# pingooio/pingoo

Measured on AMD Instinct MI355X. Metric: requests/sec matched (whole node), 1k-rule WAF, higher is better.
Workload: dtype u8

## Files before the change

include/pwaf.h:

```cpp
#ifndef PWAF_H
#define PWAF_H

#include <stddef.h>
#include <stdint.h>

#ifdef __cplusplus
extern "C" {
#endif

#define PWAF_ABI_VERSION 4u

#define PWAF_OK 0
#define PWAF_E_INVALID_ARG (-1)
#define PWAF_E_SYNTAX (-2)
#define PWAF_E_UNSUPPORTED (-3)
#define PWAF_E_LIST (-4)
#define PWAF_E_DEVICE (-5)
#define PWAF_E_BATCH (-6)
#define PWAF_E_NOMEM (-7)
#define PWAF_E_BUSY (-8)
#define PWAF_W_PARTIAL 1

#define PWAF_ACTION_ALLOW 0u
#define PWAF_ACTION_BLOCK 1u
// ... 275 lines not shown
    float ms;
    uint64_t alg_bytes;
} pwaf_kernel_time;
int pwaf_engine_set_profiling(pwaf_engine *, int on);
int pwaf_engine_kernel_times(pwaf_engine *, pwaf_kernel_time *out, int cap);

typedef struct pwaf_stats {
    uint32_t n_rules, n_atoms, n_scan_atoms, n_numeric_atoms;
    uint32_t n_dfa_groups, n_dfa_states_total, max_dfa_states, dfa_table_bytes_total;
    uint32_t n_ip_lists, ipset_trie_nodes, geo_trie_nodes, n_dnf_literals;
    uint32_t n_warnings, n_filtered_groups ,
        n_gated_groups ,
        n_confirm_literals ;
} pwaf_stats;
int pwaf_engine_stats(const pwaf_engine *, pwaf_stats *out);
int pwaf_engine_rule_errors(pwaf_engine *, uint64_t *counts, size_t n_rules);
int pwaf_engine_residual_mode(const pwaf_engine *);
const char *pwaf_engine_residual_fallback(const pwaf_engine *);
size_t pwaf_program_residual_source(const pwaf_program *, int kind, char *buf, size_t cap);
long pwaf_program_residual_compile(const pwaf_program *, const char *arch, char *err, size_t err_len);
int pwaf_program_confirm_field(const pwaf_program *, uint32_t group, const uint8_t *bytes, size_t len, uint32_t arena_offset,
                               uint16_t *atoms, size_t cap, size_t *n_atoms, int *flagged, int *walk);
int pwaf_engine_address_tables(const pwaf_engine *, uint32_t out[8]);
int pwaf_program_stats(const pwaf_program *, pwaf_stats *out);

size_t pwaf_derive_path(const uint8_t *uri_path, size_t len);
void pwaf_derive_user_agent(const uint8_t *hdr, size_t len, int present, size_t *out_start, size_t *out_len);
void pwaf_derive_host(const uint8_t *uri_host, size_t uri_host_len, int uri_host_present,
                      const uint8_t *host_hdr, size_t host_hdr_len, int host_hdr_present,
                      int *out_from_header, size_t *out_start, size_t *out_len);

const char *pwaf_last_error(void);
uint32_t pwaf_abi_version(void);

#ifdef __cplusplus
}
#endif
#endif
```

pingoo_amd/_abi.py:

```python
import ctypes as C

ABI_VERSION = 4

OK = 0
E_INVALID_ARG = -1
E_SYNTAX = -2
E_UNSUPPORTED = -3
E_LIST = -4
E_DEVICE = -5
E_BATCH = -6
E_NOMEM = -7
E_BUSY = -8

ACTION_ALLOW, ACTION_BLOCK, ACTION_CAPTCHA, ACTION_BYPASS = 0, 1, 2, 3
RULE_NONE = 0xFFFFFFFF
RULE_UA_GATE = 0xFFFFFFFE
RULE_CAPTCHA_ENDPOINT = 0xFFFFFFFD
RULE_ACTION_BLOCK, RULE_ACTION_CAPTCHA = 1, 2

LIST_STRING, LIST_INT, LIST_IP = 0, 1, 2
OPT_NO_UA_GATE, OPT_NO_CAPTCHA_BYPASS, OPT_NO_PREFILTER, OPT_STRICT, OPT_FILTER_STRIDE2, OPT_LENIENT, OPT_NO_RESIDUAL, OPT_GLOBAL_VERDICT_TABLES, OPT_NO_CONFIRM, OPT_NO_RESIDUAL_JIT = 1, 2, 4, 8, 16, 32, 64, 128, 512, 1024
OPT_DENSE_VERDICT, OPT_TINY_VERDICT_SLOTS, OPT_NO_DIR_SUMMARY, OPT_SPARSE_VERDICT, OPT_EAGER_CMP, OPT_NO_DENSE_SWITCH = 2048, 4096, 8192, 16384, 32768, 65536
OPT_GEO_ANSWERS = 256
OPT_RULE_HITS = 131072
W_PARTIAL = 1
MEM_HOST, MEM_DEVICE = 0, 1
FLAG_CAPTCHA_VERIFIED = 1
N_FIELDS = 5
FIELD_NAMES = ("host", "url", "path", "method", "user_agent")
ARENA_PAD = 16
ADDRESS_TABLE_FIELDS = ("escapes", "n_vals", "has_summary", "shift", "common", "packed", "classes", "sets")
GEO_ANSWER_TABLE_FIELDS = ("has_table", "escapes", "n_vals", "has_summary", "shift", "common", "records", "zero")


class RuleDesc(C.Structure):
    _fields_ = [
        ("name", C.c_char_p),
        ("expression", C.c_char_p),
        ("actions", C.POINTER(C.c_uint8)),
        ("n_actions", C.c_uint32),
        ("reserved", C.c_uint32),
    ]


class ListDesc(C.Structure):
    _fields_ = [
        ("name", C.c_char_p),
        ("type", C.c_uint32),
        ("n_items", C.c_uint32),
        ("items", C.POINTER(C.c_char_p)),
    ]


class GeoipEntry(C.Structure):
# ... 173 lines not shown
```

pingoo_amd/csrc/dirtable.h:

```cpp
#pragma once
#include <cstddef>
#include <cstdint>
#include <unordered_map>
#include <vector>

namespace pwaf {
namespace dirtable {

static constexpr uint32_t kChunkWords = 32;
static constexpr size_t kEntries = (size_t)1 << 24;

struct Compressed {
    std::vector<uint32_t> chunks;
    std::vector<uint32_t> vals;
    std::vector<uint32_t> summary;
    uint32_t shift = 0, common = 0;
};

inline void compress(const uint32_t *d24, bool no_summary, Compressed &out) {
    out.chunks.assign((size_t)65536 * kChunkWords, 0);
    out.vals.clear();
    out.summary.clear();
    out.shift = out.common = 0;
    for (uint32_t x = 0; x < 65536; x++) {
        const uint32_t *en = &d24[(size_t)x << 8];
        for (uint32_t w = 0; w < 8; w++) {
            uint32_t *rec = &out.chunks[(size_t)x * kChunkWords + 4 * w];
            uint32_t bm = 0, n_starts = 0;
            for (uint32_t j = 32 * w; j < 32 * w + 32; j++)
                if (j == 0 || en[j] != en[j - 1]) {
                    bm |= 1u << (j & 31);
                    if (n_starts == 1) rec[3] = (uint32_t)out.vals.size();
                    if (n_starts == 0) rec[2] = en[j];
                    else out.vals.push_back(en[j]);
                    n_starts++;
                }
            rec[0] = bm;
            rec[1] = w ? en[32 * w - 1] : 0u;
        }
    }
    if (out.vals.empty()) out.vals.push_back(0);
    if (no_summary) return;
    std::unordered_map<uint32_t, uint64_t> run_len;
    for (size_t x = 0; x < kEntries;) {
        size_t y = x + 1;
        while (y < kEntries && d24[y] == d24[x]) y++;
// ... 4 lines not shown
    uint64_t best_len = 0;
    for (const auto &kv : run_len)
        if (kv.second > best_len || (kv.second == best_len && kv.first < common)) { common = kv.first; best_len = kv.second; }
    double best_cost = 1e9;
    uint32_t best_shift = 0;
    std::vector<uint32_t> best_bits;
    for (uint32_t shift = 0; shift <= 4; shift++) {
        const size_t n_blk = kEntries >> shift;
        std::vector<uint32_t> bits(n_blk / 32, 0);
        uint64_t set = 0;
        for (size_t b = 0; b < n_blk; b++) {
            bool other = false;
            for (size_t j = b << shift; j < ((b + 1) << shift) && !other; j++) other = d24[j] != common;
            if (other) { bits[b >> 5] |= 1u << (b & 31); set++; }
        }
        const double cost = (double)set / (double)n_blk + (double)(n_blk / 8) / (8.0 * 1024 * 1024);
        if (cost < best_cost && set * 2 <= n_blk) { best_cost = cost; best_shift = shift; best_bits.swap(bits); }
    }
    if (!best_bits.empty()) {
        out.summary.swap(best_bits);
        out.shift = best_shift;
        out.common = common;
    }
}

}
}
```

pingoo_amd/csrc/engine.cpp:

```cpp
#include <hip/hip_runtime_api.h>

#include <cstdio>
#include <algorithm>
#include <cstring>
#include <map>
#include <memory>
#include <mutex>
#include <string>
#include <type_traits>
#include <unordered_map>
#include <vector>

#include "dirtable.h"
#include "georec.h"
#include "frontend.h"
#include "kernels.h"
#include "lscan_split.h"
#include "program.h"
#include "records.h"

using namespace pwaf;

struct pwaf_program {
    std::unique_ptr<Program> p;
// ... 230 lines not shown
    uint32_t cmp_vars = 0;
    uint32_t cc_words = 1, n_cmp_atoms = 0, n_bit_atoms = 0, n_trig = 0, n_lazy = 0;
    DevBuf lazy_atoms;
    std::vector<uint32_t> lazy_vars;
    uint32_t n_short = 0;
    int short_field = -1;
    DevBuf short_atoms;
    uint32_t class_words = 1, acmp_words = 0, geo_default = 0, n_classes = 1;
    DevBuf class_rows, dir_esc, leaf_root, geo_leaf_root;
    std::vector<uint32_t> host_cc_masks, host_iu_masks1;
    std::vector<std::pair<uint32_t, uint32_t>> host_acmp;
    std::vector<int64_t> host_iu_vals1;
    DevBuf iu_vals[2], iu_masks[2];
    uint32_t iu_n[2] = {0, 0}, iu_words[2] = {1, 1};
    DevBuf ip_root4, ip_root6, ip_nodes, geo_root4, geo_root6, geo_nodes, geo_recs;
    std::mutex mu;
    std::mutex prof_mu;
    DevBuf residual_errors;
    std::string residual_note;
    JitKernel residual_jit;
    DevBuf residual_blob, geo_rec_root4, geo_rec_root6, geo_rec_nodes;
    DevBuf pass_base, colmask, dir24 , dir_chunks, dir_vals, dir_summary;
    uint32_t dir_sum_shift = 0, dir_common = 0;
    uint32_t dir_n_esc = 0, dir_n_vals = 0;
    bool geo_answers = false;
    DevBuf georec_chunks, georec_vals, georec_summary;
    uint32_t georec_shift = 0, georec_common = 0, georec_n_esc = 0, georec_n_vals = 0;
    uint32_t n_need = 0;
    uint32_t n_visit = 0;
    std::vector<double> mean_len;
    uint32_t n_ungated = 0, n_gated = 0, n_filtered = 0;
    std::vector<uint8_t> owns_factors;
    uint32_t n_gap = 0;
    std::vector<uint32_t> lscan_launches[2];
    DevBuf pass_table;
    std::vector<uint32_t> hlen_fields;
    uint32_t n_fields = PWAF_N_FIELDS;
    int profiling = 0;
    std::vector<hipEvent_t> ev;
    std::vector<pwaf_kernel_time> times;
    std::vector<std::pair<size_t, size_t>> time_ev;
    size_t n_timed = 0;
    uint32_t n_cus = 256;
};

namespace {
// ... 247 lines not shown
}

void set_trie_args(const pwaf_engine *e, VerdictArgs &v) {
    const Program &P = *e->prog.p;
    const uint32_t *leaf = (const uint32_t *)e->leaf_root.p;
    v.ip_root4 = P.ipset_trie.root4.empty() ? leaf : (const uint32_t *)e->ip_root4.p;
    v.ip_root6 = P.ipset_trie.root6.empty() ? leaf : (const uint32_t *)e->ip_root6.p;
    v.ip_nodes = (const uint32_t *)e->ip_nodes.p;
    v.set_masks = (const uint32_t *)e->set_masks.p;
    v.set_words = P.set_words;
    v.n_ip_lists = P.n_ip_lists;
    const uint32_t *geo_leaf = (const uint32_t *)e->geo_leaf_root.p;
    v.geo_root4 = P.geo_trie.root4.empty() ? geo_leaf : (const uint32_t *)e->geo_root4.p;
    v.geo_root6 = P.geo_trie.root6.empty() ? geo_leaf : (const uint32_t *)e->geo_root6.p;
    v.geo_nodes = (const uint32_t *)e->geo_nodes.p;
    v.has_geo = P.has_geo ? 1u : 0u;
    v.dir24 = (const uint32_t *)e->dir24.p;
    v.dir_chunks = (const uint32_t *)e->dir_chunks.p;
    v.dir_vals = (const uint32_t *)e->dir_vals.p;
    v.dir_esc = (const uint2 *)e->dir_esc.p;
    v.dir_summary = (const uint32_t *)e->dir_summary.p;
    v.dir_sum_shift = e->dir_sum_shift;
    v.dir_common = e->dir_common;
    v.class_rows = (const uint32_t *)e->class_rows.p;
    v.class_words = e->class_words;
    v.acmp_words = e->acmp_words;
    v.geo_default = e->geo_default;
    const size_t n_sets = P.set_words ? P.set_masks.size() / P.set_words : 1;
    v.ipres_packed = (e->n_classes <= 65536u && n_sets <= 65536u) ? 1u : 0u;
}

void set_georec_args(const pwaf_engine *e, GeoRecArgs &g) {
    g.has_geo = e->prog.p->has_geo ? 1u : 0u;
    g.root4 = (const uint32_t *)e->geo_rec_root4.p;
    g.root6 = (const uint32_t *)e->geo_rec_root6.p;
    g.nodes = (const uint32_t *)e->geo_rec_nodes.p;
    g.recs = (const GeoRec *)e->geo_recs.p;
    g.chunks = (const uint32_t *)e->georec_chunks.p;
    g.vals = (const uint32_t *)e->georec_vals.p;
    g.summary = (const uint32_t *)e->georec_summary.p;
    g.sum_shift = e->georec_shift;
    g.common = e->georec_common;
    g.n_cus = e->n_cus;
}
int need_geo_answers(const pwaf_engine *e, const char *fn) {
    if (e->geo_answers) return PWAF_OK;
// ... 1491 lines not shown
        if (P.has_geo && P.residual_needs_geo) {
            const std::vector<uint32_t> leaf0(65536, TRIE_LEAF);
            UP(geo_rec_root4, (P.geo_trie.root4.empty() ? leaf0 : P.geo_trie.root4))
            UP(geo_rec_root6, (P.geo_trie.root6.empty() ? leaf0 : P.geo_trie.root6))
            UP(geo_rec_nodes, P.geo_trie.nodes)
            UP(geo_recs, P.geo_recs)
        }
    }
#undef UP
    if (P.flags & PWAF_OPT_GEO_ANSWERS) {
        e->geo_answers = true;
        const std::vector<uint32_t> leaf0(65536, TRIE_LEAF);
        if (!e->geo_rec_root4.p) {
            if ((rc = upload(e->geo_rec_root4, P.geo_trie.root4.empty() ? leaf0 : P.geo_trie.root4)) || (rc = upload(e->geo_rec_root6, P.geo_trie.root6.empty() ? leaf0 : P.geo_trie.root6)) ||
                (rc = upload(e->geo_rec_nodes, P.geo_trie.nodes)))
                return dev_fail(rc);
            const std::vector<GeoRec> def{GeoRec{0u, (uint16_t)('X' | ('X' << 8)), 0u}};
            if ((rc = upload(e->geo_recs, P.geo_recs.empty() ? def : P.geo_recs))) return dev_fail(rc);
        }
        if (P.has_geo && !P.geo_trie.root4.empty()) {
            std::vector<uint32_t> d24;
            e->georec_n_esc = georec::flatten(P.geo_trie.root4.data(), P.geo_trie.nodes.data(), d24);
            dirtable::Compressed ct;
            dirtable::compress(d24.data(), (P.flags & PWAF_OPT_NO_DIR_SUMMARY) != 0, ct);
            if ((rc = upload(e->georec_chunks, ct.chunks)) || (rc = upload(e->georec_vals, ct.vals))) return dev_fail(rc);
            if (!ct.summary.empty()) {
                if ((rc = upload(e->georec_summary, ct.summary))) return dev_fail(rc);
                e->georec_shift = ct.shift;
                e->georec_common = ct.common;
            }
            e->georec_n_vals = (uint32_t)ct.vals.size();
        }
    }
    if ((P.has_geo && !P.geo_trie.root4.empty()) || (P.n_ip_lists && !P.ipset_trie.root4.empty())) {
        VerdictArgs tv{};
        set_trie_args(e.get(), tv);
        DevBuf cnt;
        if ((rc = cnt.reserve(4))) return dev_fail(rc);
        uint32_t n_esc = 0;
        bool ok = hipMemset(cnt.p, 0, 4) == hipSuccess && launch_dir24(tv, nullptr, nullptr, cnt.p, nullptr) == 0 &&
                  hipMemcpy(&n_esc, cnt.p, 4, hipMemcpyDeviceToHost) == hipSuccess;
        if (ok) ok = e->dir24.reserve((size_t)4 << 24) == PWAF_OK && e->dir_esc.reserve((size_t)std::max(1u, n_esc) * 8) == PWAF_OK;
        if (ok) ok = hipMemset(cnt.p, 0, 4) == hipSuccess && launch_dir24(tv, e->dir24.p, e->dir_esc.p, cnt.p, nullptr) == 0 && hipDeviceSynchronize() == hipSuccess;
        cnt.release();
        if (!ok) { fail(PWAF_E_DEVICE, "DIR-24 table build failed"); return dev_fail(PWAF_E_DEVICE); }
        {
            std::vector<uint32_t> d24((size_t)1 << 24);
            if (hipMemcpy(d24.data(), e->dir24.p, d24.size() * 4, hipMemcpyDeviceToHost) != hipSuccess) { fail(PWAF_E_DEVICE, "DIR-24 download failed"); return dev_fail(PWAF_E_DEVICE); }
            static_assert(dirtable::kChunkWords == kDirChunkWords, "dirtable.h and kernels.h disagree on the record layout");
            dirtable::Compressed ct;
            dirtable::compress(d24.data(), (P.flags & PWAF_OPT_NO_DIR_SUMMARY) != 0, ct);
            if ((rc = upload(e->dir_chunks, ct.chunks)) || (rc = upload(e->dir_vals, ct.vals))) return dev_fail(rc);
            if (!ct.summary.empty()) {
                if ((rc = upload(e->dir_summary, ct.summary))) return dev_fail(rc);
                e->dir_sum_shift = ct.shift;
                e->dir_common = ct.common;
            }
            e->dir_n_esc = n_esc;
            e->dir_n_vals = (uint32_t)ct.vals.size();
            e->dir24.release();
        }
    }
    if (hipDeviceSynchronize() != hipSuccess) { fail(PWAF_E_DEVICE, "device synchronize failed after table upload"); return dev_fail(PWAF_E_DEVICE); }
    *out = e.release();
    return partial;
}

void pwaf_engine_destroy(pwaf_engine *e) {
    if (!e) return;
    for (auto &g : e->groups) { for (DevBuf *b : {&g.tab, &g.classmap, &g.special, &g.list_off, &g.list, &g.ftable, &g.c_head, &g.c_entries, &g.c_bytes, &g.c_classes}) b->release(); g.fl.release(); g.rt.release(); }
    for (DevBuf *b : {&e->num_atoms, &e->lazy_atoms, &e->bit_atoms, &e->trig_off, &e->trig_rules, &e->always_rules, &e->iu_vals[0], &e->iu_vals[1], &e->iu_masks[0], &e->iu_masks[1], &e->country_luts, &e->rules, &e->lits,
                      &e->set_masks, &e->ip_root4, &e->ip_root6, &e->ip_nodes, &e->geo_root4, &e->geo_root6, &e->geo_nodes, &e->geo_recs, &e->residual_blob, &e->residual_errors, &e->geo_rec_root4, &e->geo_rec_root6, &e->geo_rec_nodes, &e->pass_base, &e->colmask, &e->dir24, &e->dir_chunks, &e->dir_vals, &e->dir_summary, &e->class_rows,
                      &e->dir_esc, &e->leaf_root, &e->geo_leaf_root, &e->pass_table, &e->georec_chunks, &e->georec_vals, &e->georec_summary})
        b->release();
    if (e->residual_jit.module) {
        int cur = -1;
        const bool have = hipGetDevice(&cur) == hipSuccess;
        (void)hipSetDevice(e->device);
        jit_release(e->residual_jit);
        if (have) (void)hipSetDevice(cur);
    }
    for (auto &c : e->ctx) c->release();
    for (auto ev : e->ev) (void)hipEventDestroy(ev);
    delete e;
}

int pwaf_engine_residual_mode(const pwaf_engine *e) {
    if (!e || e->prog.p->n_residual == 0) return 0;
    return e->residual_jit.function ? 2 : 1;
}
const char *pwaf_engine_residual_fallback(const pwaf_engine *e) { return e ? e->residual_note.c_str() : ""; }
int pwaf_engine_address_tables(const pwaf_engine *e, uint32_t out[8]) {
    if (!e || !out) return fail(PWAF_E_INVALID_ARG, "pwaf_engine_address_tables: NULL argument");
    const Program &P = *e->prog.p;
    VerdictArgs v{};
    set_trie_args(e, v);
    out[0] = e->dir_n_esc;
    out[1] = e->dir_chunks.p ? e->dir_n_vals : 0u;
    out[2] = e->dir_summary.p ? 1u : 0u;
    out[3] = e->dir_sum_shift;
    out[4] = e->dir_common;
    out[5] = v.ipres_packed;
    out[6] = e->n_classes;
    out[7] = P.set_words ? (uint32_t)(P.set_masks.size() / P.set_words) : 1u;
    return PWAF_OK;
}
int pwaf_engine_geo_answer_tables(const pwaf_engine *e, uint32_t out[8]) {
    if (!e || !out) return fail(PWAF_E_INVALID_ARG, "pwaf_engine_geo_answer_tables: NULL argument");
    if (int rc = need_geo_answers(e, "pwaf_engine_geo_answer_tables")) return rc;
    out[0] = e->georec_chunks.p ? 1u : 0u;
    out[1] = e->georec_n_esc;
    out[2] = e->georec_chunks.p ? e->georec_n_vals : 0u;
    out[3] = e->georec_summary.p ? 1u : 0u;
    out[4] = e->georec_shift;
    out[5] = e->georec_common;
    out[6] = (uint32_t)std::max<size_t>(1, e->prog.p->geo_recs.size());
    out[7] = 0;
    return PWAF_OK;
}
size_t pwaf_program_residual_source(const pwaf_program *p, int kind, char *buf, size_t cap) {
    if (!p || p->p->n_residual == 0) return 0;
    std::string text, why;
    const std::vector<uint8_t> &blob = p->p->residual_blob;
    if (!(kind == 0 ? rvm_specialize(blob.data(), blob.size(), text, why) : rvm_jit_program(blob.data(), blob.size(), text, why))) {
        (void)fail(PWAF_E_UNSUPPORTED, why);
        return 0;
    }
// ... 914 lines not shown
```

pingoo_amd/csrc/kernels.h:

```cpp
#pragma once
#include <cstdint>
#include <string>
#include <vector>

#include "program.h"

namespace pwaf {

static constexpr int kMaxPasses = 250;
static constexpr int kVerdictPre = 12;
static constexpr uint32_t kGapLists = 32;
static constexpr uint32_t kMaxHeaderLens = 8;
static constexpr uint32_t kDirChunkWords = 32;

static constexpr uint32_t REC_OVERFLOW = 0x80000000u;
struct PoolEntry {
    uint32_t atom;
    uint32_t next;
};

struct SpecialCell {
    uint32_t next_off;
    uint32_t emit;
};
// ... 278 lines not shown
    uint32_t lazy_var[4], n_lazy_var;
    const uint32_t *bit_col;
    const int64_t *iu_vals[2];
    const uint32_t *iu_masks[2];
    uint32_t iu_n[2], iu_words[2];
    const uint32_t *country_masks;
    uint32_t cc_words;
    const DevRule *rules;
    uint32_t n_rules;
    const uint32_t *lits;
    uint32_t n_lits, n_trig;
    const uint32_t *trig_off;
    const uint16_t *trig_rules;
    const uint32_t *always_rules;
    const uint32_t *ip_root4, *ip_root6, *ip_nodes;
    const uint32_t *set_masks;
    uint32_t set_words;
    uint32_t n_ip_lists;
    const uint32_t *geo_root4, *geo_root6, *geo_nodes;
    const uint32_t *dir24;
    const uint32_t *dir_chunks, *dir_vals;
    const uint32_t *dir_summary;
    uint32_t dir_sum_shift, dir_common;
    const uint2 *dir_esc;
    const uint32_t *class_rows;
    uint32_t class_words;
    uint32_t acmp_words;
    uint32_t geo_default;
    uint32_t *ipres;
    uint32_t ipres_packed;
    uint32_t has_geo;
    uint4 *gpairs;
    uint32_t *ghdr;
    uint32_t pair_stride;
    uint32_t attr_blocks;
    pwaf_verdict *out;
    unsigned long long *counts;
    uint32_t *match_idx;
    uint32_t *n_matches;
    pwaf_rule_hit *hits;
    uint32_t hits_cap;
    uint32_t *n_hits;
    unsigned long long *rule_hits;
};

int launch_scan(const ScanArgs &a, void *stream);
struct GatedTable {
    const ListScanArgs *g;
    uint32_t count;
    uint32_t debug;
};
struct ListShape {
    uint32_t threads, hot_bytes, wg_per_cu;
};
ListShape list_shape(uint32_t variant);
uint32_t list_hot_bytes(const ListShape &shape);
int launch_scan_gated(const ListScanArgs *host, uint32_t count, const ListScanArgs *dev, uint32_t *plan, const ListShape &shape, void *stream);
int launch_verdict(const VerdictArgs &a, void *stream);
int launch_ipres(const VerdictArgs &a, void *stream);
int launch_attr(const VerdictArgs &a, void *stream);
int launch_dir24(const VerdictArgs &a, void *out , void *esc, void *esc_count, void *stream);
struct GeoRecArgs {
    const uint8_t *ip, *ip_is_v6;
    const uint32_t *asn;
    const uint16_t *country;
    uint32_t n, has_geo;
    const uint32_t *root4, *root6, *nodes;
    const GeoRec *recs;
    const uint32_t *chunks, *vals, *summary;
    uint32_t sum_shift, common;
    uint32_t n_cus;
    uint2 *out;
};
int launch_georec(const GeoRecArgs &a, void *stream);
uint32_t scan_lds_bytes(uint32_t n_hot, uint32_t stride, uint32_t n_gate_atoms);
struct VerdictShape {
    uint32_t waves, lds_bytes, lds_tables;
    uint32_t sparse, v_cap, per_cu;
};
VerdictShape verdict_shape(uint32_t n_cols, uint32_t n_rules, uint32_t n_trig, uint32_t n_lits, bool force_global = false, int mode = 3, uint32_t n_passes = 0);
uint32_t verdict_blocks_sp(const VerdictShape &sh, uint32_t n_cus);

// ... 2 lines not shown
```

pingoo_amd/csrc/kernels.hip:

```cpp
#include <hip/hip_runtime.h>

#include <cstdlib>
#include <mutex>
#include <set>

#include "confirm.h"
#include "utf8.h"
#include "kernels.h"
#include "residual.h"

namespace pwaf {

static constexpr int kScanThreads = 1024;
static constexpr int kScanWaves = kScanThreads / 64;
static constexpr uint32_t kNone = 0xFFFFFFFFu;

#define PWAF_LDS __attribute__((address_space(3)))
#define PWAF_GLOBAL __attribute__((address_space(1)))
typedef const PWAF_LDS uint16_t *lds_u16_ptr;
typedef const PWAF_GLOBAL uint16_t *glb_u16_ptr;
typedef const PWAF_LDS uint32_t *lds_u32_ptr;
typedef const PWAF_LDS uint8_t *lds_u8_ptr;
typedef unsigned int u32x4 __attribute__((ext_vector_type(4)));
typedef u32x4 u32x4_u __attribute__((aligned(1)));
// ... 2744 lines not shown
        __builtin_amdgcn_fence(__ATOMIC_ACQ_REL, "wavefront");
        if (HITS && q_n != 0 && ++q_k == 0x10000u) q_flush();
        cur = nxt;
    }
    if (HITS && a.n_hits != nullptr) q_flush();
    __syncthreads();
    unsigned long long *tally = reinterpret_cast<unsigned long long *>(lds);
    if (lane == 0) {
        tally[wave * 4 + PWAF_ACTION_ALLOW] = cnt_allow;
        tally[wave * 4 + PWAF_ACTION_BLOCK] = cnt_block;
        tally[wave * 4 + PWAF_ACTION_CAPTCHA] = cnt_captcha;
        tally[wave * 4 + PWAF_ACTION_BYPASS] = cnt_bypass;
    }
    __syncthreads();
    if (a.counts != nullptr && tid < 4) {
        unsigned long long sum = 0;
        for (uint32_t wv = 0; wv < n_waves; wv++) sum += tally[wv * 4 + tid];
        if (sum) atomicAdd(&a.counts[tid], sum);
    }
}

static constexpr uint32_t DIR_ESCAPE = 0x80000000u;

template <bool PACKED>
__global__ __launch_bounds__(256) void ipres_kernel(VerdictArgs a) {
    constexpr uint32_t U = 4;
    const bool from_row = a.asn == nullptr;
#ifdef PWAF_PROFILING
    const bool dir = a.dir_chunks != nullptr && !((a.debug_skip >> 16) & 1u);
    const bool skip_v6 = (a.debug_skip >> 17) & 1u, skip_v4 = (a.debug_skip >> 16) & 1u;
#else
    const bool dir = a.dir_chunks != nullptr;
    constexpr bool skip_v6 = false, skip_v4 = false;
#endif
    const uint32_t T = gridDim.x * 256u;
    for (uint32_t i0 = blockIdx.x * 256u + threadIdx.x; i0 < a.n; i0 += T * U) {
        uint32_t idx[U], ipw[U][4], eg[U], ei[U], k[U];
        bool live[U], v6[U], geo_walk[U], chunked[U];
        uint4 raw[U];
        uint32_t v6b[U];
#pragma unroll
        for (uint32_t u = 0; u < U; u++) {
            idx[u] = i0 + u * T;
            live[u] = idx[u] < a.n;
            const uint32_t j = live[u] ? idx[u] : i0;
            raw[u] = *reinterpret_cast<const uint4 *>(a.ip + (size_t)j * 16);
            v6b[u] = a.ip_is_v6[j];
        }
        uint32_t first[U], top16[U];
#pragma unroll
        for (uint32_t u = 0; u < U; u++) {
            ipw[u][0] = raw[u].x; ipw[u][1] = raw[u].y; ipw[u][2] = raw[u].z; ipw[u][3] = raw[u].w;
            v6[u] = v6b[u] != 0;
            geo_walk[u] = false;
            if (from_row && a.has_geo) {
                if (!v6[u]) {
                    const uint32_t b0 = ipw[u][0] & 0xFFu;
                    geo_walk[u] = !(b0 == 127u || (b0 & 0xF0u) == 0xE0u);
                } else {
                    const bool loopback = ipw[u][0] == 0 && ipw[u][1] == 0 && ipw[u][2] == 0 && ipw[u][3] == 0x01000000u;
                    geo_walk[u] = !(loopback || (ipw[u][0] & 0xFFu) == 0xFFu);
                }
            }
            top16[u] = (ip_byte(ipw[u], 0) << 8) | ip_byte(ipw[u], 1);
            eg[u] = ei[u] = TRIE_LEAF;
            chunked[u] = !v6[u] && dir;
            first[u] = 0;
            if (!chunked[u] && !(v6[u] ? skip_v6 : skip_v4)) {
                if (geo_walk[u]) eg[u] = (v6[u] ? a.geo_root6 : a.geo_root4)[top16[u]];
                if (a.n_ip_lists) ei[u] = (v6[u] ? a.ip_root6 : a.ip_root4)[top16[u]];
            }
        }
        uint32_t look[U];
#pragma unroll
        for (uint32_t u = 0; u < U; u++) {
            look[u] = chunked[u] ? 1u : 0u;
            if (chunked[u] && a.dir_summary != nullptr) {
                const uint32_t blk = ((top16[u] << 8) | ip_byte(ipw[u], 2)) >> a.dir_sum_shift;
                look[u] = (a.dir_summary[blk >> 5] >> (blk & 31u)) & 1u;
            }
        }
        uint4 rec4[U];
#pragma unroll
        for (uint32_t u = 0; u < U; u++) {
            rec4[u] = make_uint4(0u, 0u, 0u, 0u);
            if (look[u]) rec4[u] = *reinterpret_cast<const uint4 *>(a.dir_chunks + (size_t)top16[u] * kDirChunkWords + 4u * (ip_byte(ipw[u], 2) >> 5));
        }
        uint32_t e24[U];
#pragma unroll
        for (uint32_t u = 0; u < U; u++) {
            e24[u] = a.dir_common;
            if (look[u]) {
                const uint32_t rank = (uint32_t)__builtin_popcount(rec4[u].x & (0xFFFFFFFFu >> (31u - (ip_byte(ipw[u], 2) & 31u))));
                e24[u] = rank == 0 ? rec4[u].y : rank == 1 ? rec4[u].z : a.dir_vals[rec4[u].w + rank - 2u];
            }
        }
#pragma unroll
        for (uint32_t u = 0; u < U; u++) {
            k[u] = 2;
            if (!v6[u] && dir) {
// ... 394 lines not shown
    const uint32_t x = blockIdx.x * 256 + threadIdx.x;
    if (x >= (1u << 24)) return;
    uint32_t eg = a.geo_root4[x >> 8];
    if (!(eg & TRIE_LEAF)) eg = a.geo_nodes[(size_t)eg * 256 + (x & 0xFFu)];
    uint32_t ei = a.ip_root4[x >> 8];
    if (!(ei & TRIE_LEAF)) ei = a.ip_nodes[(size_t)ei * 256 + (x & 0xFFu)];
    const uint32_t vg = eg & ~TRIE_LEAF, vi = ei & ~TRIE_LEAF;
    if ((eg & ei & TRIE_LEAF) && vg < 65536u && vi < 32768u) {
        if (out) out[x] = vg | (vi << 16);
        return;
    }
    const uint32_t idx = atomicAdd(esc_count, 1u);
    if (esc) {
        esc[idx] = make_uint2(eg, ei);
        out[x] = DIR_ESCAPE | idx;
    }
}

int launch_dir24(const VerdictArgs &a, void *out, void *esc, void *esc_count, void *stream) {
    hipLaunchKernelGGL(dir24_kernel, dim3((1u << 24) / 256), dim3(256), 0, (hipStream_t)stream, a, (uint32_t *)out, (uint2 *)esc, (uint32_t *)esc_count);
    return (int)hipGetLastError();
}

int launch_ipres(const VerdictArgs &a, void *stream) {
    if (a.n == 0) return 0;
#ifdef PWAF_PROFILING
    static const uint32_t forced = getenv("PWAF_IPRES_BLOCKS") ? (uint32_t)atoi(getenv("PWAF_IPRES_BLOCKS")) : 0u;
#else
    const uint32_t forced = 0;
#endif
    const uint32_t blocks = std::min<uint32_t>((a.n + 255) / 256, forced ? forced : 8 * std::max(1u, a.attr_blocks));
    if (a.ipres_packed) hipLaunchKernelGGL(ipres_kernel<true>, dim3(blocks), dim3(256), 0, (hipStream_t)stream, a);
    else hipLaunchKernelGGL(ipres_kernel<false>, dim3(blocks), dim3(256), 0, (hipStream_t)stream, a);
    return (int)hipGetLastError();
}

int launch_georec(const GeoRecArgs &a, void *stream) {
    if (a.n == 0) return 0;
    const uint32_t blocks = std::min<uint32_t>((a.n + 255) / 256, 8 * std::max(1u, a.n_cus));
    hipLaunchKernelGGL(georec_kernel, dim3(blocks), dim3(256), 0, (hipStream_t)stream, a);
    return (int)hipGetLastError();
}

int launch_attr(const VerdictArgs &a, void *stream) {
    if (a.n == 0) return 0;
#ifdef PWAF_PROFILING
    static const uint32_t forced = getenv("PWAF_ATTR_BLOCKS") ? (uint32_t)atoi(getenv("PWAF_ATTR_BLOCKS")) : 0u;
#else
    const uint32_t forced = 0;
#endif
    const uint32_t blocks = std::min<uint32_t>((a.n_groups + 3) / 4, forced ? forced : 6 * std::max(1u, a.attr_blocks));
    const bool small = a.set_words <= 4 && a.cc_words <= 2 && a.iu_words[0] <= 1 && a.iu_words[1] <= 1 && a.acmp_words <= 1;
    if (a.ipres_packed && small) hipLaunchKernelGGL((attr_kernel<true, true>), dim3(blocks), dim3(256), 0, (hipStream_t)stream, a);
    else if (a.ipres_packed) hipLaunchKernelGGL((attr_kernel<true, false>), dim3(blocks), dim3(256), 0, (hipStream_t)stream, a);
    else if (small) hipLaunchKernelGGL((attr_kernel<false, true>), dim3(blocks), dim3(256), 0, (hipStream_t)stream, a);
    else hipLaunchKernelGGL((attr_kernel<false, false>), dim3(blocks), dim3(256), 0, (hipStream_t)stream, a);
// ... 142 lines not shown
```

pingoo_amd/engine.py:

```python
from __future__ import annotations

import ctypes as C
import enum
import ipaddress
import os
from dataclasses import dataclass, field
from typing import Dict, Iterable, List, Optional, Sequence, Tuple

import numpy as np

from . import _abi
from .batch import GEO_DTYPE, RULE_HIT_DTYPE, VERDICT_DTYPE, Request, RequestBatch

_LIB = None
_LIB_PATH = os.path.join(os.path.dirname(os.path.abspath(__file__)), f"libpwaf_{os.environ['PWAF_LIB_VARIANT']}.so" if os.environ.get("PWAF_LIB_VARIANT") else "libpwaf.so")


class PwafError(RuntimeError):
    def __init__(self, code: int, message: str, rule_index: Optional[int] = None):
        super().__init__(f"[{code}] {message}")
        self.code = code
        self.message = message
        self.rule_index = rule_index

# ... 95 lines not shown
    L.pwaf_batcher_destroy.argtypes = [vp]
    L.pwaf_batcher_destroy.restype = None
    L.pwaf_evaluate_records.argtypes = [vp, vp, C.c_size_t, vp, C.c_uint32, vp, vp]
    L.pwaf_async_create.argtypes = [vp, C.c_uint32, C.c_uint32, C.c_uint32, C.POINTER(vp)]
    L.pwaf_async_submit.argtypes = [vp, C.POINTER(_abi.Request), C.c_uint64]
    L.pwaf_async_poll.argtypes = [vp, C.POINTER(_abi.Completion), C.c_size_t]
    L.pwaf_async_poll.restype = C.c_size_t
    L.pwaf_async_fd.argtypes = [vp]
    L.pwaf_async_flush.argtypes = [vp]
    L.pwaf_async_stats.argtypes = [vp, C.POINTER(C.c_uint64), C.POINTER(C.c_uint64), C.POINTER(C.c_uint64)]
    L.pwaf_async_destroy.argtypes = [vp]
    L.pwaf_async_destroy.restype = None
    L.pwaf_geoip_lookup.argtypes = [vp, vp, vp, C.c_uint32, C.c_uint32, vp, vp]
    L.pwaf_evaluate_batch_geo.argtypes = [vp, C.POINTER(_abi.Batch), vp, vp, vp]
    L.pwaf_evaluate_device_geo.argtypes = [vp, C.POINTER(_abi.Batch), vp, vp, vp, vp, vp, vp]
    L.pwaf_evaluate_batch_hits.argtypes = [vp, C.POINTER(_abi.Batch), vp, vp, vp, C.c_uint32, vp, vp]
    L.pwaf_evaluate_device_hits.argtypes = [vp, C.POINTER(_abi.Batch), vp, vp, vp, vp, vp, C.c_uint32, vp, vp, vp]
    L.pwaf_evaluate_records_geo.argtypes = [vp, vp, C.c_size_t, vp, C.c_uint32, vp, vp, vp]
    L.pwaf_evaluate_one_geo.argtypes = [vp, C.POINTER(_abi.Request), C.POINTER(_abi.Verdict), C.POINTER(_abi.Geo)]
    L.pwaf_async_create_geo.argtypes = [vp, C.c_uint32, C.c_uint32, C.c_uint32, C.POINTER(vp)]
    L.pwaf_async_poll_geo.argtypes = [vp, C.POINTER(_abi.Completion), C.POINTER(_abi.Geo), C.c_size_t]
    L.pwaf_async_poll_geo.restype = C.c_size_t
    L.pwaf_engine_geo_answer_tables.argtypes = [vp, C.POINTER(C.c_uint32)]
    L.pwaf_geoip_from_mmdb.argtypes = [C.c_char_p, C.c_size_t, C.POINTER(C.POINTER(_abi.GeoipEntry)), C.POINTER(C.c_size_t)]
    L.pwaf_geoip_from_file_image.argtypes = [C.c_char_p, C.c_char_p, C.c_size_t, C.POINTER(C.POINTER(_abi.GeoipEntry)), C.POINTER(C.c_size_t)]
    L.pwaf_zstd_decompress.argtypes = [C.c_char_p, C.c_size_t, C.POINTER(C.c_void_p), C.POINTER(C.c_size_t)]
    L.pwaf_buffer_free.argtypes = [C.c_void_p]
    L.pwaf_buffer_free.restype = None
    L.pwaf_geoip_free.argtypes = [C.POINTER(_abi.GeoipEntry)]
    L.pwaf_geoip_free.restype = None
    L.pwaf_list_parse_csv.argtypes = [C.c_char_p, C.c_size_t, C.POINTER(C.POINTER(C.c_char_p)), C.POINTER(C.c_size_t)]
    L.pwaf_list_free.argtypes = [C.POINTER(C.c_char_p), C.c_size_t]
    L.pwaf_list_free.restype = None
    L.pwaf_engine_kernel_times.argtypes = [vp, C.POINTER(_abi.KernelTime), C.c_int]
    L.pwaf_derive_path.argtypes = [C.c_char_p, C.c_size_t]
    L.pwaf_derive_path.restype = C.c_size_t
    L.pwaf_derive_user_agent.argtypes = [C.c_char_p, C.c_size_t, C.c_int, C.POINTER(C.c_size_t), C.POINTER(C.c_size_t)]
    L.pwaf_derive_user_agent.restype = None
    L.pwaf_derive_host.argtypes = [C.c_char_p, C.c_size_t, C.c_int, C.c_char_p, C.c_size_t, C.c_int, C.POINTER(C.c_int), C.POINTER(C.c_size_t), C.POINTER(C.c_size_t)]
    L.pwaf_derive_host.restype = None
    if L.pwaf_abi_version() != _abi.ABI_VERSION:
        raise ImportError("libpwaf.so ABI version mismatch: rebuild with `python -m pingoo_amd.build --force`")
    _LIB = L
    return L


# ... 193 lines not shown
            self._h = None

    def __del__(self):
        self.close()

    @property
    def program(self) -> CompiledProgram:
        return CompiledProgram._borrow(lib().pwaf_engine_program(self._h))

    @property
    def residual_mode(self) -> int:
        return int(lib().pwaf_engine_residual_mode(self._h))

    @property
    def residual_fallback(self) -> str:
        return (lib().pwaf_engine_residual_fallback(self._h) or b"").decode(errors="replace")

    def address_tables(self) -> dict:
        out = (C.c_uint32 * len(_abi.ADDRESS_TABLE_FIELDS))()
        rc = lib().pwaf_engine_address_tables(self._h, out)
        if rc != 0:
            _raise(rc, lib().pwaf_last_error().decode(errors="replace"))
        return dict(zip(_abi.ADDRESS_TABLE_FIELDS, (int(x) for x in out)))

    def geo_answer_tables(self) -> dict:
        out = (C.c_uint32 * len(_abi.GEO_ANSWER_TABLE_FIELDS))()
        rc = lib().pwaf_engine_geo_answer_tables(self._h, out)
        if rc != 0:
            _raise(rc, lib().pwaf_last_error().decode(errors="replace"))
        return dict(zip(_abi.GEO_ANSWER_TABLE_FIELDS, (int(x) for x in out)))

    def lookup_geoip(self, ip16, v6) -> np.ndarray:
        ip16 = np.ascontiguousarray(ip16, dtype=np.uint8).reshape(-1, 16)
        v6 = np.ascontiguousarray(v6, dtype=np.uint8).reshape(-1)
        assert len(ip16) == len(v6)
        out = np.zeros(len(v6), dtype=GEO_DTYPE)
        rc = lib().pwaf_geoip_lookup(self._h, ip16.ctypes.data, v6.ctypes.data, len(v6), _abi.MEM_HOST, out.ctypes.data, None)
        if rc != 0:
            _raise(rc, lib().pwaf_last_error().decode(errors="replace"))
        return out

    def rule_errors(self, n_rules: int) -> List[int]:
        arr = (C.c_uint64 * n_rules)()
        rc = lib().pwaf_engine_rule_errors(self._h, arr, n_rules)
        if rc != 0:
            _raise(rc, lib().pwaf_last_error().decode(errors="replace"))
# ... 547 lines not shown
```

Measured before the change: 7.462 billion.

## Add LDS-resident coarse occupancy bitmap to prefilter DIR-24 IP lookups

Builds a coarser bitmap over the DIR-24 summary at compile time, sized to fit a shared-memory budget, and uploads it. The ipres kernel gains a COARSE variant that loads this bitmap into LDS once per workgroup, runs with 1024-thread workgroups, and checks LDS before touching the global summary and chunk tables. Input loads for the first iteration are issued before the LDS fill to overlap latency. This trades a per-block LDS fill and lower occupancy options for fewer global memory probes on IPs in empty regions. A stats accessor exposes the new table parameters.

New measurement: 7.595 billion (median of 6 runs). 1.8% higher.

```diff
diff --git a/include/pwaf.h b/include/pwaf.h
--- a/include/pwaf.h
+++ b/include/pwaf.h
@@ -321,6 +321,7 @@
 int pwaf_program_confirm_field(const pwaf_program *, uint32_t group, const uint8_t *bytes, size_t len, uint32_t arena_offset,
                                uint16_t *atoms, size_t cap, size_t *n_atoms, int *flagged, int *walk);
 int pwaf_engine_address_tables(const pwaf_engine *, uint32_t out[8]);
+int pwaf_engine_coarse_tables(const pwaf_engine *, uint32_t out[16]);
 int pwaf_program_stats(const pwaf_program *, pwaf_stats *out);
 
 size_t pwaf_derive_path(const uint8_t *uri_path, size_t len);
diff --git a/pingoo_amd/_abi.py b/pingoo_amd/_abi.py
--- a/pingoo_amd/_abi.py
+++ b/pingoo_amd/_abi.py
@@ -30,6 +30,8 @@
 FIELD_NAMES = ("host", "url", "path", "method", "user_agent")
 ARENA_PAD = 16
 ADDRESS_TABLE_FIELDS = ("escapes", "n_vals", "has_summary", "shift", "common", "packed", "classes", "sets")
+COARSE_TABLE_FIELDS = ("present", "shift", "bytes", "blocks_set", "summary_blocks_set", "threads", "wg_per_cu", "zero7",
+                       "rec_present", "rec_shift", "rec_bytes", "rec_blocks_set", "zero12", "zero13", "zero14", "zero15")
 GEO_ANSWER_TABLE_FIELDS = ("has_table", "escapes", "n_vals", "has_summary", "shift", "common", "records", "zero")
 
 
diff --git a/pingoo_amd/csrc/dirtable.h b/pingoo_amd/csrc/dirtable.h
--- a/pingoo_amd/csrc/dirtable.h
+++ b/pingoo_amd/csrc/dirtable.h
@@ -15,13 +15,25 @@
     std::vector<uint32_t> vals;
     std::vector<uint32_t> summary;
     uint32_t shift = 0, common = 0;
+    std::vector<uint32_t> coarse;
+    uint32_t coarse_shift = 0;
 };
 
-inline void compress(const uint32_t *d24, bool no_summary, Compressed &out) {
+static constexpr size_t kCoarseBudget = 64 * 1024;
+static constexpr uint32_t kMaxCoarseShift = 12;
+
+inline uint64_t popcount_words(const std::vector<uint32_t> &w) {
+    uint64_t n = 0;
+    for (uint32_t x : w) n += (uint64_t)__builtin_popcount(x);
+    return n;
+}
+
+inline void compress(const uint32_t *d24, bool no_summary, Compressed &out, size_t coarse_budget = kCoarseBudget) {
     out.chunks.assign((size_t)65536 * kChunkWords, 0);
     out.vals.clear();
     out.summary.clear();
-    out.shift = out.common = 0;
+    out.coarse.clear();
+    out.shift = out.common = out.coarse_shift = 0;
     for (uint32_t x = 0; x < 65536; x++) {
         const uint32_t *en = &d24[(size_t)x << 8];
         for (uint32_t w = 0; w < 8; w++) {
@@ -72,6 +84,26 @@
         out.shift = best_shift;
         out.common = common;
     }
+    if (out.summary.empty()) return;
+    for (uint32_t cs = out.shift + 1; cs <= kMaxCoarseShift; cs++) {
+        const size_t n_blk = kEntries >> cs;
+        if (n_blk / 8 > coarse_budget) continue;
+        const uint32_t per = 1u << (cs - out.shift);
+        std::vector<uint32_t> bits(n_blk / 32, 0);
+        uint64_t set = 0;
+        for (size_t b = 0; b < n_blk; b++) {
+            bool any = false;
+            if (per >= 32) {
+                for (size_t w = b * (per / 32); w < (b + 1) * (per / 32) && !any; w++) any = out.summary[w] != 0;
+            } else {
+                const size_t first = b * per;
+                any = ((out.summary[first >> 5] >> (first & 31)) & ((1u << per) - 1u)) != 0;
+            }
+            if (any) { bits[b >> 5] |= 1u << (b & 31); set++; }
+        }
+        if (set * 2 <= n_blk) { out.coarse.swap(bits); out.coarse_shift = cs; }
+        break;
+    }
 }
 
 }
diff --git a/pingoo_amd/csrc/engine.cpp b/pingoo_amd/csrc/engine.cpp
--- a/pingoo_amd/csrc/engine.cpp
+++ b/pingoo_amd/csrc/engine.cpp
@@ -276,6 +276,8 @@
     DevBuf residual_blob, geo_rec_root4, geo_rec_root6, geo_rec_nodes;
     DevBuf pass_base, colmask, dir24 , dir_chunks, dir_vals, dir_summary;
     uint32_t dir_sum_shift = 0, dir_common = 0;
+    DevBuf dir_coarse;
+    uint32_t dir_coarse_shift = 0, dir_coarse_bytes = 0, dir_coarse_set = 0, dir_summary_set = 0;
     uint32_t dir_n_esc = 0, dir_n_vals = 0;
     bool geo_answers = false;
     DevBuf georec_chunks, georec_vals, georec_summary;
@@ -569,6 +571,9 @@
     v.dir_summary = (const uint32_t *)e->dir_summary.p;
     v.dir_sum_shift = e->dir_sum_shift;
     v.dir_common = e->dir_common;
+    v.dir_coarse = (const uint32_t *)e->dir_coarse.p;
+    v.dir_coarse_shift = e->dir_coarse_shift;
+    v.dir_coarse_bytes = e->dir_coarse_bytes;
     v.class_rows = (const uint32_t *)e->class_rows.p;
     v.class_words = e->class_words;
     v.acmp_words = e->acmp_words;
@@ -2106,7 +2111,7 @@
             std::vector<uint32_t> d24;
             e->georec_n_esc = georec::flatten(P.geo_trie.root4.data(), P.geo_trie.nodes.data(), d24);
             dirtable::Compressed ct;
-            dirtable::compress(d24.data(), (P.flags & PWAF_OPT_NO_DIR_SUMMARY) != 0, ct);
+            dirtable::compress(d24.data(), (P.flags & PWAF_OPT_NO_DIR_SUMMARY) != 0, ct, 0);
             if ((rc = upload(e->georec_chunks, ct.chunks)) || (rc = upload(e->georec_vals, ct.vals))) return dev_fail(rc);
             if (!ct.summary.empty()) {
                 if ((rc = upload(e->georec_summary, ct.summary))) return dev_fail(rc);
@@ -2133,12 +2138,19 @@
             if (hipMemcpy(d24.data(), e->dir24.p, d24.size() * 4, hipMemcpyDeviceToHost) != hipSuccess) { fail(PWAF_E_DEVICE, "DIR-24 download failed"); return dev_fail(PWAF_E_DEVICE); }
             static_assert(dirtable::kChunkWords == kDirChunkWords, "dirtable.h and kernels.h disagree on the record layout");
             dirtable::Compressed ct;
-            dirtable::compress(d24.data(), (P.flags & PWAF_OPT_NO_DIR_SUMMARY) != 0, ct);
+            dirtable::compress(d24.data(), (P.flags & PWAF_OPT_NO_DIR_SUMMARY) != 0, ct, ipres_shape().coarse_bytes);
             if ((rc = upload(e->dir_chunks, ct.chunks)) || (rc = upload(e->dir_vals, ct.vals))) return dev_fail(rc);
             if (!ct.summary.empty()) {
                 if ((rc = upload(e->dir_summary, ct.summary))) return dev_fail(rc);
                 e->dir_sum_shift = ct.shift;
                 e->dir_common = ct.common;
+                e->dir_summary_set = (uint32_t)dirtable::popcount_words(ct.summary);
+            }
+            if (!ct.coarse.empty()) {
+                if ((rc = upload(e->dir_coarse, ct.coarse))) return dev_fail(rc);
+                e->dir_coarse_shift = ct.coarse_shift;
+                e->dir_coarse_bytes = (uint32_t)(ct.coarse.size() * 4);
+                e->dir_coarse_set = (uint32_t)dirtable::popcount_words(ct.coarse);
             }
             e->dir_n_esc = n_esc;
             e->dir_n_vals = (uint32_t)ct.vals.size();
@@ -2154,7 +2166,7 @@
     if (!e) return;
     for (auto &g : e->groups) { for (DevBuf *b : {&g.tab, &g.classmap, &g.special, &g.list_off, &g.list, &g.ftable, &g.c_head, &g.c_entries, &g.c_bytes, &g.c_classes}) b->release(); g.fl.release(); g.rt.release(); }
     for (DevBuf *b : {&e->num_atoms, &e->lazy_atoms, &e->bit_atoms, &e->trig_off, &e->trig_rules, &e->always_rules, &e->iu_vals[0], &e->iu_vals[1], &e->iu_masks[0], &e->iu_masks[1], &e->country_luts, &e->rules, &e->lits,
-                      &e->set_masks, &e->ip_root4, &e->ip_root6, &e->ip_nodes, &e->geo_root4, &e->geo_root6, &e->geo_nodes, &e->geo_recs, &e->residual_blob, &e->residual_errors, &e->geo_rec_root4, &e->geo_rec_root6, &e->geo_rec_nodes, &e->pass_base, &e->colmask, &e->dir24, &e->dir_chunks, &e->dir_vals, &e->dir_summary, &e->class_rows,
+                      &e->set_masks, &e->ip_root4, &e->ip_root6, &e->ip_nodes, &e->geo_root4, &e->geo_root6, &e->geo_nodes, &e->geo_recs, &e->residual_blob, &e->residual_errors, &e->geo_rec_root4, &e->geo_rec_root6, &e->geo_rec_nodes, &e->pass_base, &e->colmask, &e->dir24, &e->dir_chunks, &e->dir_vals, &e->dir_summary, &e->dir_coarse, &e->class_rows,
                       &e->dir_esc, &e->leaf_root, &e->geo_leaf_root, &e->pass_table, &e->georec_chunks, &e->georec_vals, &e->georec_summary})
         b->release();
     if (e->residual_jit.module) {
@@ -2187,6 +2199,19 @@
     out[5] = v.ipres_packed;
     out[6] = e->n_classes;
     out[7] = P.set_words ? (uint32_t)(P.set_masks.size() / P.set_words) : 1u;
+    return PWAF_OK;
+}
+int pwaf_engine_coarse_tables(const pwaf_engine *e, uint32_t out[16]) {
+    if (!e || !out) return fail(PWAF_E_INVALID_ARG, "pwaf_engine_coarse_tables: NULL argument");
+    const IpresShape sh = ipres_shape();
+    for (int i = 0; i < 16; i++) out[i] = 0;
+    out[0] = e->dir_coarse.p ? 1u : 0u;
+    out[1] = e->dir_coarse_shift;
+    out[2] = e->dir_coarse_bytes;
+    out[3] = e->dir_coarse_set;
+    out[4] = e->dir_summary_set;
+    out[5] = e->dir_coarse.p ? sh.threads : 256u;
+    out[6] = e->dir_coarse.p ? sh.wg_per_cu : 8u;
     return PWAF_OK;
 }
 int pwaf_engine_geo_answer_tables(const pwaf_engine *e, uint32_t out[8]) {
diff --git a/pingoo_amd/csrc/kernels.h b/pingoo_amd/csrc/kernels.h
--- a/pingoo_amd/csrc/kernels.h
+++ b/pingoo_amd/csrc/kernels.h
@@ -324,6 +324,8 @@
     const uint32_t *dir_chunks, *dir_vals;
     const uint32_t *dir_summary;
     uint32_t dir_sum_shift, dir_common;
+    const uint32_t *dir_coarse;
+    uint32_t dir_coarse_shift, dir_coarse_bytes;
     const uint2 *dir_esc;
     const uint32_t *class_rows;
     uint32_t class_words;
@@ -360,6 +362,10 @@
 int launch_scan_gated(const ListScanArgs *host, uint32_t count, const ListScanArgs *dev, uint32_t *plan, const ListShape &shape, void *stream);
 int launch_verdict(const VerdictArgs &a, void *stream);
 int launch_ipres(const VerdictArgs &a, void *stream);
+struct IpresShape {
+    uint32_t threads, coarse_bytes, wg_per_cu;
+};
+IpresShape ipres_shape();
 int launch_attr(const VerdictArgs &a, void *stream);
 int launch_dir24(const VerdictArgs &a, void *out , void *esc, void *esc_count, void *stream);
 struct GeoRecArgs {
diff --git a/pingoo_amd/csrc/kernels.hip b/pingoo_amd/csrc/kernels.hip
--- a/pingoo_amd/csrc/kernels.hip
+++ b/pingoo_amd/csrc/kernels.hip
@@ -2790,9 +2790,10 @@
 
 static constexpr uint32_t DIR_ESCAPE = 0x80000000u;
 
-template <bool PACKED>
-__global__ __launch_bounds__(256) void ipres_kernel(VerdictArgs a) {
+template <bool PACKED, bool COARSE>
+__global__ __launch_bounds__(COARSE ? 1024 : 256, COARSE ? 8 : 1) void ipres_kernel(VerdictArgs a) {
     constexpr uint32_t U = 4;
+    extern __shared__ uint4 ipres_lds[];
     const bool from_row = a.asn == nullptr;
 #ifdef PWAF_PROFILING
     const bool dir = a.dir_chunks != nullptr && !((a.debug_skip >> 16) & 1u);
@@ -2801,19 +2802,43 @@
     const bool dir = a.dir_chunks != nullptr;
     constexpr bool skip_v6 = false, skip_v4 = false;
 #endif
-    const uint32_t T = gridDim.x * 256u;
-    for (uint32_t i0 = blockIdx.x * 256u + threadIdx.x; i0 < a.n; i0 += T * U) {
+    const uint32_t T = gridDim.x * blockDim.x;
+    uint32_t i0 = blockIdx.x * blockDim.x + threadIdx.x;
+    uint4 raw[U];
+    uint32_t v6b[U];
+    auto load_inputs = [&](uint32_t base) {
+#pragma unroll
+        for (uint32_t u = 0; u < U; u++) {
+            const uint32_t j = base + u * T < a.n ? base + u * T : base;
+            raw[u] = *reinterpret_cast<const uint4 *>(a.ip + (size_t)j * 16);
+            v6b[u] = a.ip_is_v6[j];
+        }
+    };
+    bool loaded = false;
+    if (COARSE) {
+        load_inputs(i0 < a.n ? i0 : 0u);
+        loaded = true;
+        const uint4 *src = reinterpret_cast<const uint4 *>(a.dir_coarse);
+        const uint32_t n16 = a.dir_coarse_bytes >> 4;
+        for (uint32_t j = threadIdx.x; j < n16; j += 4u * blockDim.x) {
+            uint4 w[4];
+#pragma unroll
+            for (uint32_t q = 0; q < 4; q++) w[q] = src[min(j + q * blockDim.x, n16 - 1u)];
+#pragma unroll
+            for (uint32_t q = 0; q < 4; q++)
+                if (j + q * blockDim.x < n16) ipres_lds[j + q * blockDim.x] = w[q];
+        }
+        __syncthreads();
+    }
+    for (; i0 < a.n; i0 += T * U) {
         uint32_t idx[U], ipw[U][4], eg[U], ei[U], k[U];
         bool live[U], v6[U], geo_walk[U], chunked[U];
-        uint4 raw[U];
-        uint32_t v6b[U];
+        if (!loaded) load_inputs(i0);
+        loaded = false;
 #pragma unroll
         for (uint32_t u = 0; u < U; u++) {
             idx[u] = i0 + u * T;
             live[u] = idx[u] < a.n;
-            const uint32_t j = live[u] ? idx[u] : i0;
-            raw[u] = *reinterpret_cast<const uint4 *>(a.ip + (size_t)j * 16);
-            v6b[u] = a.ip_is_v6[j];
         }
         uint32_t first[U], top16[U];
 #pragma unroll
@@ -2843,7 +2868,14 @@
 #pragma unroll
         for (uint32_t u = 0; u < U; u++) {
             look[u] = chunked[u] ? 1u : 0u;
-            if (chunked[u] && a.dir_summary != nullptr) {
+            if (COARSE && chunked[u]) {
+                const uint32_t blk = ((top16[u] << 8) | ip_byte(ipw[u], 2)) >> a.dir_coarse_shift;
+                look[u] = (reinterpret_cast<const uint32_t *>(ipres_lds)[blk >> 5] >> (blk & 31u)) & 1u;
+            }
+        }
+#pragma unroll
+        for (uint32_t u = 0; u < U; u++) {
+            if (look[u] && a.dir_summary != nullptr) {
                 const uint32_t blk = ((top16[u] << 8) | ip_byte(ipw[u], 2)) >> a.dir_sum_shift;
                 look[u] = (a.dir_summary[blk >> 5] >> (blk & 31u)) & 1u;
             }
@@ -3284,6 +3316,19 @@
     return (int)hipGetLastError();
 }
 
+#ifndef PWAF_IPRES_SHAPE
+#define PWAF_IPRES_SHAPE 1
+#endif
+IpresShape ipres_shape() {
+    static const IpresShape shapes[4] = {{256, 0, 8}, {1024, 64 * 1024, 2}, {512, 32 * 1024, 4}, {1024, 64 * 1024, 1}};
+#ifdef PWAF_PROFILING
+    static const uint32_t pick = getenv("PWAF_IPRES_SHAPE") ? (uint32_t)atoi(getenv("PWAF_IPRES_SHAPE")) & 3u : (uint32_t)PWAF_IPRES_SHAPE;
+#else
+    const uint32_t pick = PWAF_IPRES_SHAPE;
+#endif
+    return shapes[pick];
+}
+
 int launch_ipres(const VerdictArgs &a, void *stream) {
     if (a.n == 0) return 0;
 #ifdef PWAF_PROFILING
@@ -3291,9 +3336,17 @@
 #else
     const uint32_t forced = 0;
 #endif
+    if (a.dir_coarse != nullptr) {
+        const IpresShape sh = ipres_shape();
+        if (a.dir_coarse_shift > 17u || a.dir_coarse_bytes != (1u << 21) >> a.dir_coarse_shift || a.dir_coarse_bytes > sh.coarse_bytes) return (int)hipErrorInvalidValue;
+        const uint32_t blocks = std::min<uint32_t>((a.n + sh.threads - 1) / sh.threads, forced ? forced : sh.wg_per_cu * std::max(1u, a.attr_blocks));
+        if (a.ipres_packed) hipLaunchKernelGGL((ipres_kernel<true, true>), dim3(blocks), dim3(sh.threads), a.dir_coarse_bytes, (hipStream_t)stream, a);
+        else hipLaunchKernelGGL((ipres_kernel<false, true>), dim3(blocks), dim3(sh.threads), a.dir_coarse_bytes, (hipStream_t)stream, a);
+        return (int)hipGetLastError();
+    }
     const uint32_t blocks = std::min<uint32_t>((a.n + 255) / 256, forced ? forced : 8 * std::max(1u, a.attr_blocks));
-    if (a.ipres_packed) hipLaunchKernelGGL(ipres_kernel<true>, dim3(blocks), dim3(256), 0, (hipStream_t)stream, a);
-    else hipLaunchKernelGGL(ipres_kernel<false>, dim3(blocks), dim3(256), 0, (hipStream_t)stream, a);
+    if (a.ipres_packed) hipLaunchKernelGGL((ipres_kernel<true, false>), dim3(blocks), dim3(256), 0, (hipStream_t)stream, a);
+    else hipLaunchKernelGGL((ipres_kernel<false, false>), dim3(blocks), dim3(256), 0, (hipStream_t)stream, a);
     return (int)hipGetLastError();
 }
 
diff --git a/pingoo_amd/engine.py b/pingoo_amd/engine.py
--- a/pingoo_amd/engine.py
+++ b/pingoo_amd/engine.py
@@ -141,6 +141,7 @@
     L.pwaf_async_poll_geo.argtypes = [vp, C.POINTER(_abi.Completion), C.POINTER(_abi.Geo), C.c_size_t]
     L.pwaf_async_poll_geo.restype = C.c_size_t
     L.pwaf_engine_geo_answer_tables.argtypes = [vp, C.POINTER(C.c_uint32)]
+    L.pwaf_engine_coarse_tables.argtypes = [vp, C.POINTER(C.c_uint32)]
     L.pwaf_geoip_from_mmdb.argtypes = [C.c_char_p, C.c_size_t, C.POINTER(C.POINTER(_abi.GeoipEntry)), C.POINTER(C.c_size_t)]
     L.pwaf_geoip_from_file_image.argtypes = [C.c_char_p, C.c_char_p, C.c_size_t, C.POINTER(C.POINTER(_abi.GeoipEntry)), C.POINTER(C.c_size_t)]
     L.pwaf_zstd_decompress.argtypes = [C.c_char_p, C.c_size_t, C.POINTER(C.c_void_p), C.POINTER(C.c_size_t)]
@@ -380,6 +381,13 @@
         if rc != 0:
             _raise(rc, lib().pwaf_last_error().decode(errors="replace"))
         return dict(zip(_abi.ADDRESS_TABLE_FIELDS, (int(x) for x in out)))
+
+    def coarse_tables(self) -> dict:
+        out = (C.c_uint32 * len(_abi.COARSE_TABLE_FIELDS))()
+        rc = lib().pwaf_engine_coarse_tables(self._h, out)
+        if rc != 0:
+            _raise(rc, lib().pwaf_last_error().decode(errors="replace"))
+        return dict(zip(_abi.COARSE_TABLE_FIELDS, (int(x) for x in out)))
 
     def geo_answer_tables(self) -> dict:
         out = (C.c_uint32 * len(_abi.GEO_ANSWER_TABLE_FIELDS))()
```
